# Plonky3/Plonky3-recursion

Hardware: AMD Instinct MI355X
Metric: prove_next_layer ms + Poseidon2 perms/s, KoalaBear 2^20-row circuit, 1/8 GPU (lower is better)
Workload: dtype u32 Montgomery (31-bit prime field, degree-4 extension); Poseidon2 hashing as exact integers in f64; 1 GPU; prove_next_layer (verifier-circuit run on the device + prove_all_tables) of the synthetic koala-bear 2^20-row recursion layer: tables const/public/alu/poseidon2/recompose, FRI blowup 4, arity<=4, 54 queries, 15-bit PoW; circuit inputs + NextLayerPrepCache resident in HBM; field=koala-bear, log_height=20, independent_proofs=1, proof_bytes=612900, parallelism=1 independent proofs, one per GPU, no data-path collective

## Files before the change

### __graft_entry__.py

```python
import os
import subprocess
import sys
import time

ROOT = os.path.dirname(os.path.abspath(__file__))
CSRC = os.path.join(ROOT, "plonky3_recursion_amd", "csrc")
LIB = os.path.join(ROOT, "plonky3_recursion_amd", "libp3r_hip.so")
KNOBS_LIB = os.path.join(ROOT, "plonky3_recursion_amd", "knobs", "libp3r_hip.so")
HIP_SOURCES = ["p3r_core.hip", "tu_lde.hip", "tu_open.hip", "tu_fri.hip", "tu_quotient.hip", "tu_logup.hip", "tu_mmcs4.hip", "prep_device.hip"]


def _stale(target, deps):
    if not os.path.exists(target):
        return True
    t = os.path.getmtime(target)
    return any(os.path.getmtime(d) > t for d in deps)


def _deps_of(obj):
    dep = obj + ".d"
    if not os.path.exists(dep):
        return None
    txt = open(dep).read().replace("\\\n", " ")
    return [p for p in txt.split(":", 1)[1].split() if p]


def build():
    hipcc = os.environ.get("HIPCC", "/opt/rocm/bin/hipcc")
    flags = ["-O3", "-std=c++17", "--offload-arch=gfx950", "-fPIC", "-pthread"]
    objdir = os.path.join(CSRC, ".build")
    os.makedirs(objdir, exist_ok=True)
    os.makedirs(os.path.dirname(KNOBS_LIB), exist_ok=True)
    shared = ["prep_device.hip", "tu_open.hip", "tu_fri.hip", "tu_quotient.hip", "tu_logup.hip", "tu_mmcs4.hip"]
    knobbed = ["p3r_core.hip", "tu_lde.hip"]
    units = [(src, src + ".o", []) for src in HIP_SOURCES]
    units += [(src, src.replace(".hip", ".knobs.o"), ["-DP3R_TUNING_KNOBS"]) for src in knobbed]
    test_only = ["tu_prims_test.hip", "tu_p2f_test.hip", "tu_field_test.hip"]
    units += [(src, src.replace(".hip", ".knobs.o"), ["-DP3R_TUNING_KNOBS"]) for src in test_only]
    pending = []
    for src, objname, extra in units:
        obj = os.path.join(objdir, objname)
        deps = _deps_of(obj)
        if deps is None or not all(os.path.exists(d) for d in deps) or _stale(obj, deps):
            pending.append((obj, [hipcc] + flags + extra + ["-MD", "-MF", obj + ".d", "-c", "-o", obj, os.path.join(CSRC, src)]))
    pending.sort(key=lambda job: 0 if "p3r_core" in os.path.basename(job[0]) else 1)
    running, failed = [], None
    max_jobs = max(1, min(len(pending), (os.cpu_count() or 2)))
    while pending or running:
        while pending and len(running) < max_jobs:
            obj, cmd = pending.pop(0)
            running.append((obj, subprocess.Popen(cmd, cwd=CSRC)))
        done = [job for job in running if job[1].poll() is not None]
# ... 104 lines not shown
```

### plonky3_recursion_amd/csrc/circuit_impl.hip.h

```cpp

#include "circuit_host.h"

namespace {

template <class PP, int D = 4>
__device__ __forceinline__ typename CircuitExt<PP, D>::type w_load(const uint32_t* __restrict__ w, uint32_t id) {
  typename CircuitExt<PP, D>::type e;
  if constexpr (D == 4) {
    const uint4 v = *reinterpret_cast<const uint4*>(w + (size_t)id * 4);
    e.c[0] = Fp<PP>::raw(v.x); e.c[1] = Fp<PP>::raw(v.y); e.c[2] = Fp<PP>::raw(v.z); e.c[3] = Fp<PP>::raw(v.w);
  } else {
#pragma unroll
    for (int k = 0; k < D; ++k) e.c[k] = Fp<PP>::raw(w[(size_t)id * D + k]);
  }
  return e;
}
template <class PP, int D = 4>
__device__ __forceinline__ void w_store(uint32_t* __restrict__ w, uint32_t id, const typename CircuitExt<PP, D>::type& e) {
  if constexpr (D == 4) {
    *reinterpret_cast<uint4*>(w + (size_t)id * 4) = make_uint4(e.c[0].v, e.c[1].v, e.c[2].v, e.c[3].v);
  } else {
#pragma unroll
    for (int k = 0; k < D; ++k) w[(size_t)id * D + k] = e.c[k].v;
  }
// ... 24 lines not shown
struct RunArgs {
  const RunOp* light;
  const RunP2* p2;
  const RunP2B* p2b;
  uint32_t* w;
  const uint32_t* ext;
  uint32_t* alu_values;
  uint32_t* rec_values;
  uint32_t* p2_inputs;
  size_t p2_h;
  uint8_t* p2_flags;
  uint32_t* p2_seed;
  uint32_t* p2_out;
  const int32_t* pd_slot;
  const uint32_t* siblings;
  const uint32_t* rc;
  const uint32_t* diag;
  uint32_t* err;
  const uint32_t* light_off;
  const RunSchedule::P2Seg* p2segs;
  const uint32_t* p2seg_off;
  const RunP2W* p2w;
  uint32_t* p2w_inputs;
  size_t p2w_h;
  uint8_t* p2w_flags;
  uint32_t* p2w_out;
  const int32_t* pdw_slot;
  const uint32_t* siblings_w;
  const uint32_t* rcw;
  const RunSchedule::P2Seg* p2wsegs;
  const uint32_t* p2wseg_off;
};
// ... 92 lines not shown
      }
      w_put<PP, D>(w, op.out, v, chk_out, err, op.op_idx);
      break;
    }
    default: break;
  }
}

template <class PP>
__device__ __forceinline__ void run_p2_segment(const RunArgs& A, RunSchedule::P2Seg seg, int j, bool live) {
  using F = Fp<PP>;
  using E = Fp4<PP>;
  uint32_t* __restrict__ w = A.w;
  uint32_t* err = A.err;
  if (!live) seg.n = 0;
  const CoopRc<PP> rcs = coop_load_rc<PP>(A.rc, j);
  const F diag_j = F::raw(A.diag[j]);
  F carried = F::zero();
  RunP2 next = seg.n ? A.p2[seg.first] : RunP2{};
  for (uint32_t k = 0; k < seg.n; ++k) {
    const RunP2 q = next;
    if (k + 1 < seg.n) next = A.p2[seg.first + k + 1];
    const bool new_start = q.flags & 1, merkle = q.flags & 2;
    F s = F::zero();
    if (!new_start && (!merkle || j < 8)) s = k ? carried : F::raw(A.p2_out[(size_t)q.prev_row * 16 + j]);
    const int32_t slot = A.pd_slot[q.row];
    if (merkle && slot >= 0 && j >= 8) s = F::raw(A.siblings[(size_t)slot * 8 + (j - 8)]);
    const uint32_t in_w = q.in[j >> 2];
    if (in_w != kNoW) s = F::raw(w[(size_t)in_w * 4 + (j & 3)]);
    bool bit = false;
    if (q.bit_w != kNoW) {
      const E v = w_load<PP>(w, q.bit_w);
// ... 5 lines not shown
      if (merkle && bit) s = F::raw(other);
    }
    A.p2_inputs[(size_t)j * A.p2_h + q.row] = s.v;
    if (j == 0) {
      A.p2_flags[q.row] = q.flags & 1;
      A.p2_flags[A.p2_h + q.row] = (q.flags >> 1) & 1;
      A.p2_flags[2 * A.p2_h + q.row] = bit;
      uint32_t seed = 0;
      if (q.idx_w != kNoW) {
        const E v = w_load<PP>(w, q.idx_w);
        if (v.c[1].v | v.c[2].v | v.c[3].v) run_error(err, q.op_idx, RUN_ERR_INDEX_SUM);
        seed = v.c[0].v;
      }
      A.p2_seed[q.row] = seed;
    }
    s = coop_permute<PP>(s, j, diag_j, rcs);
    carried = s;
    A.p2_out[(size_t)q.row * 16 + j] = s.v;
    const uint32_t n_out = (q.flags >> 8) & 7;
    const uint32_t l = (uint32_t)j >> 2;
    if (l < n_out && q.out[l] != kNoW) {
      uint32_t* slot_w = w + (size_t)q.out[l] * 4 + (j & 3);
      if (q.flags & (1u << (4 + l))) { if (*slot_w != s.v) run_error(err, q.op_idx, RUN_ERR_CONFLICT); }
      else *slot_w = s.v;
    }
  }
}

template <class PP>
__device__ __forceinline__ void run_p2w_segment(const RunArgs& A, RunSchedule::P2Seg seg, int j, bool live) {
  using F = Fp<PP>;
// ... 46 lines not shown
    const uint32_t l = (uint32_t)j >> 2;
    if (l < n_out && q.out[l] != kNoW) {
      uint32_t* slot_w = w + (size_t)q.out[l] * 4 + (j & 3);
      if (q.flags & (1u << (16 + l))) { if (*slot_w != s.v) run_error(err, q.op_idx, RUN_ERR_CONFLICT); }
      else *slot_w = s.v;
    }
  }
}

template <class PP, int D>
__device__ __forceinline__ void run_p2_segment_base(const RunArgs& A, RunSchedule::P2Seg seg, int j, bool live) {
  using F = Fp<PP>;
  uint32_t* __restrict__ w = A.w;
  uint32_t* err = A.err;
  if (!live) seg.n = 0;
  const CoopRc<PP> rcs = coop_load_rc<PP>(A.rc, j);
  const F diag_j = F::raw(A.diag[j]);
  F carried = F::zero();
  for (uint32_t k = 0; k < seg.n; ++k) {
    const RunP2B& q = A.p2b[seg.first + k];
    const uint32_t flags = q.flags;
    const bool new_start = flags & 1, merkle = flags & 2;
    F s = F::zero();
    if (!new_start && (!merkle || j < 8)) s = k ? carried : F::raw(A.p2_out[(size_t)q.prev_row * 16 + j]);
    const int32_t slot = A.pd_slot[q.row];
    if (merkle && slot >= 0 && j >= 8) s = F::raw(A.siblings[(size_t)slot * 8 + (j - 8)]);
    const uint32_t in_w = q.in[j];
    if (in_w != kNoW) s = F::raw(w[(size_t)in_w * D]);
    if (!merkle && j == 8 && q.absorb_len) s = s + F::from_canonical(q.absorb_len);
    bool bit = false;
    if (q.bit_w != kNoW) {
      const auto v = w_load<PP, D>(w, q.bit_w);
// ... 8 lines not shown
    A.p2_inputs[(size_t)j * A.p2_h + q.row] = s.v;
    if (j == 0) {
      A.p2_flags[q.row] = flags & 1;
      A.p2_flags[A.p2_h + q.row] = (flags >> 1) & 1;
      A.p2_flags[2 * A.p2_h + q.row] = bit;
      uint32_t seed = 0;
      if (q.idx_w != kNoW) {
        const auto v = w_load<PP, D>(w, q.idx_w);
        uint32_t high = 0;
        for (int c = 1; c < D; ++c) high |= v.c[c].v;
        if (high) run_error(err, q.op_idx, RUN_ERR_INDEX_SUM);
        seed = v.c[0].v;
      }
      A.p2_seed[q.row] = seed;
    }
    s = coop_permute<PP>(s, j, diag_j, rcs);
    carried = s;
    A.p2_out[(size_t)q.row * 16 + j] = s.v;
    const uint32_t n_out = (flags >> 8) & 31;
    if ((uint32_t)j < n_out && q.out[j] != kNoW) {
      uint32_t* slot_w = w + (size_t)q.out[j] * D;
      if (q.check_mask & (1u << j)) {
        bool same = slot_w[0] == s.v;
        for (int c = 1; c < D; ++c) same = same && slot_w[c] == 0;
        if (!same) run_error(err, q.op_idx, RUN_ERR_CONFLICT);
      } else {
        slot_w[0] = s.v;
        for (int c = 1; c < D; ++c) slot_w[c] = 0;
      }
    }
  }
// ... 512 lines not shown
    P3R_HIP(fill_async(ctx->stream, p2w_flags + p2w_h, 0, 3 * p2w_h));
    d->seed.alloc(p2w_h);
    P3R_HIP(fill_async(ctx->stream, d->seed.p, 0, p2w_h * 4));
    p2w_inputs = d->inputs->d;
    T->p2w = std::move(d);
  }
  {
    ProfScope ps(ctx, "run_levels");
    RunArgs A{};
    A.light = reinterpret_cast<const RunOp*>(C->d_light.p);
    A.p2 = reinterpret_cast<const RunP2*>(C->d_p2.p);
    A.p2b = reinterpret_cast<const RunP2B*>(C->d_p2.p);
    A.w = w.p; A.ext = C->d_ext.p; A.alu_values = T->alu_values.p; A.rec_values = T->recompose_values.p;
    A.p2_inputs = p2_inputs; A.p2_h = p2_h; A.p2_flags = p2_flags; A.p2_seed = p2_seed; A.p2_out = p2_out.p;
    A.pd_slot = reinterpret_cast<const int32_t*>(d_slot.p); A.siblings = d_sib.p;
    A.rc = ctx->rc.p; A.diag = ctx->p2_diag.p; A.err = err.p;
    A.light_off = C->d_light_off.p; A.p2seg_off = C->d_p2seg_off.p;
    A.p2segs = reinterpret_cast<const RunSchedule::P2Seg*>(C->d_p2segs.p);
    const bool has_w32 = !S.p2wseg_off.empty();
    if (has_w32) {
      A.p2w = reinterpret_cast<const RunP2W*>(C->d_p2w.p);
      A.p2w_inputs = p2w_inputs; A.p2w_h = p2w_h; A.p2w_flags = p2w_flags; A.p2w_out = p2w_out.p;
      A.pdw_slot = reinterpret_cast<const int32_t*>(in->slot_w.p); A.siblings_w = in->sib_w.p;
      A.rcw = ctx->rc.p + p2_num_constants<PP>();
      A.p2wsegs = reinterpret_cast<const RunSchedule::P2Seg*>(C->d_p2wsegs.p);
      A.p2wseg_off = C->d_p2wseg_off.p;
    }
    dispatch_ext_degree<PP>((int)ext_d, [&](auto dc) {
    constexpr int DD = decltype(dc)::value;
    for (const auto& seg : S.segments) {
      if (seg.narrow) {
// ... 110 lines not shown
```

### plonky3_recursion_amd/csrc/context.h

```cpp
#pragma once
#include <hip/hip_runtime.h>

#include <algorithm>
#include <array>
#include <atomic>
#include <cstdarg>
#include <cstdio>
#include <cstring>
#include <exception>
#include <functional>
#include <map>
#include <memory>
#include <chrono>
#include <mutex>
#include <stdexcept>
#include <string>
#include <thread>
#include <tuple>
#include <vector>

#include "../../include/p3r.h"
#include "error.h"
#include "field.h"
#include "poseidon2.h"
// ... 422 lines not shown
  p3r_config cfg{};
  std::shared_ptr<p3r::DevPool> pool = std::make_shared<p3r::DevPool>();
  bool prof_enabled = false;
  std::vector<p3r::ProfRec> prof;
  std::vector<std::pair<std::string, double>> stage_ms;
  std::string cur_stage;
  double cur_stage_t0 = 0;
  int partial_rounds = 0;
  hipStream_t stream = nullptr;
  int n_cus = 256;
  p3r::DevBuf rc;
  p3r::DevBuf rc_f64;
  const double* rcd() const { return reinterpret_cast<const double*>(rc_f64.p); }
  size_t rcd_w32_at = 0;
  const double* rcd_w32() const { return rcd() + rcd_w32_at; }
  p3r::DevBuf p2_diag;
  std::vector<uint32_t> rc_canonical;
  std::vector<uint8_t> fri_log_arities;
  p3r::ProofLayout proof_layout;
  std::vector<uint32_t> rc_mont_host;
  std::string err;
  bool w32_diag_builtin = false;
  bool w32_unacknowledged = false;
  uint64_t zk_nonce = 0;
  uint32_t zk_key[8] = {0, 0, 0, 0, 0, 0, 0, 0};
  std::vector<uint8_t> pending_proof;
  p3r::HostStage stage;
  p3r::HostLanding landing;
  p3r::HostPost post;
  std::map<std::string, p3r::DevBuf> const_tables;

// ... 19 lines not shown
```

### plonky3_recursion_amd/csrc/kernels_coop.hip.h

```cpp
#pragma once
#include "kernels.hip.h"

namespace p3r {

template <int CTRL>
__device__ __forceinline__ uint32_t dpp(uint32_t v) {
  return (uint32_t)__builtin_amdgcn_update_dpp(0, (int)v, CTRL, 0xF, 0xF, false);
}
constexpr int DPP_QUAD_NEXT1 = 0x39;
constexpr int DPP_QUAD_NEXT2 = 0x4E;
constexpr int DPP_QUAD_NEXT3 = 0x93;
constexpr int DPP_ROW_ROR1 = 0x121, DPP_ROW_ROR2 = 0x122, DPP_ROW_ROR4 = 0x124, DPP_ROW_ROR8 = 0x128;

template <class F>
__device__ __forceinline__ F coop_external(F x) {
  F b = F::raw(dpp<DPP_QUAD_NEXT1>(x.v)), c = F::raw(dpp<DPP_QUAD_NEXT2>(x.v)), d = F::raw(dpp<DPP_QUAD_NEXT3>(x.v));
  F ab = x + b;
  F y = ab.dbl() + b + (c + d);
  F t = y + F::raw(dpp<DPP_ROW_ROR4>(y.v));
  t = t + F::raw(dpp<DPP_ROW_ROR8>(t.v));
  return y + t;
}
template <class F>
__device__ __forceinline__ F coop_row_sum(F x) {
  F t = x + F::raw(dpp<DPP_ROW_ROR8>(x.v));
  t = t + F::raw(dpp<DPP_ROW_ROR4>(t.v));
  t = t + F::raw(dpp<DPP_ROW_ROR2>(t.v));
  return t + F::raw(dpp<DPP_ROW_ROR1>(t.v));
}

constexpr int DPP_QUAD_BCAST0 = 0x00;
__device__ __forceinline__ uint32_t coop_bcast0(uint32_t x0) {
  uint32_t q = dpp<DPP_QUAD_BCAST0>(x0);
  q |= dpp<DPP_ROW_ROR4>(q);
  return q | dpp<DPP_ROW_ROR8>(q);
}

template <class PP>
struct CoopRc {
  uint32_t full[2 * P2_HALF_FULL];
  uint32_t part[PP::PARTIAL_ROUNDS];
};
template <class PP>
__device__ __forceinline__ CoopRc<PP> coop_load_rc(const uint32_t* __restrict__ rc, int elem) {
  CoopRc<PP> c;
#pragma unroll
  for (int r = 0; r < P2_HALF_FULL; ++r) c.full[r] = rc[r * P2_WIDTH + elem];
#pragma unroll
  for (int r = 0; r < PP::PARTIAL_ROUNDS; ++r) c.part[r] = rc[P2_HALF_FULL * P2_WIDTH + r];
#pragma unroll
  for (int r = 0; r < P2_HALF_FULL; ++r)
    c.full[P2_HALF_FULL + r] = rc[P2_HALF_FULL * P2_WIDTH + PP::PARTIAL_ROUNDS + r * P2_WIDTH + elem];
  return c;
}

template <class PP>
__device__ __forceinline__ Fp<PP> coop_permute(Fp<PP> s, int elem, Fp<PP> diag, const CoopRc<PP>& rc) {
  using F = Fp<PP>;
  s = coop_external(s);
#pragma unroll
  for (int r = 0; r < P2_HALF_FULL; ++r) {
    s = p2_sbox<PP>(s + F::raw(rc.full[r]));
    s = coop_external(s);
  }
#pragma unroll
  for (int r = 0; r < PP::PARTIAL_ROUNDS; ++r) {
    const F rest = coop_row_sum(elem == 0 ? F::zero() : s);
    const F sb = p2_sbox<PP>(s + F::raw(rc.part[r]));
    const F sum = rest + F::raw(coop_bcast0(elem == 0 ? sb.v : 0u));
    s = (elem == 0 ? sb : s) * diag + sum;
  }
#pragma unroll
  for (int r = 0; r < P2_HALF_FULL; ++r) {
    s = p2_sbox<PP>(s + F::raw(rc.full[P2_HALF_FULL + r]));
    s = coop_external(s);
  }
  return s;
}

template <class PP>
__global__ void __launch_bounds__(kBlock)
k_mmcs_hash_rows_strided_coop(const uint32_t* const* __restrict__ cols, int wtot, size_t h, size_t stride,
                              uint32_t* __restrict__ dig, const uint32_t* __restrict__ rc,
                              const uint32_t* __restrict__ diag) {
  using F = Fp<PP>;
  const size_t gid = (size_t)blockIdx.x * kBlock + threadIdx.x;
  const size_t row = gid >> 4;
  const int e = (int)(gid & 15);
  const bool live = row < h;
  const F d = F::raw(diag[e]);
  const CoopRc<PP> rcs = coop_load_rc<PP>(rc, e);
  F s = F::zero();
  for (int g = 0; g < wtot; g += P2_RATE) {
    if (live && e < P2_RATE && g + e < wtot) s = F::raw(cols[g + e][row * stride]);
    s = coop_permute<PP>(s, e, d, rcs);
  }
  if (live && e < P2_DIGEST) dig[(size_t)e * h + row] = s.v;
}

constexpr int kSubtreeBlock = 1024;
constexpr int kSubtreeNodes = 256;
constexpr int kSubtreeLevels = 8;
struct SubtreeArgs {
  const uint32_t* in;
  uint32_t n_in;
  uint32_t local;
  int n_levels;
  uint32_t* out[kSubtreeLevels];
  const uint32_t* inj[kSubtreeLevels];
  uint32_t* t_state;
  uint32_t* t_beta;
  uint32_t* t_cap;
  int t_dc;
};

template <class PP>
__device__ __forceinline__ void fri_transcript_step(int j, uint32_t root_word, uint32_t* __restrict__ state,
                                                    uint32_t* __restrict__ beta_out, uint32_t* __restrict__ cap_out,
                                                    const CoopRc<PP>& rc, const uint32_t* __restrict__ diag, int dc = 4) {
  using F = Fp<PP>;
  F s = j < P2_RATE ? F::raw(root_word) : F::raw(state[j]);
  if (j < P2_RATE) cap_out[j] = s.v;
  if (j == P2_RATE) s += F::from_canonical(P2_RATE);
  s = coop_permute<PP>(s, j, F::raw(diag[j]), rc);
  state[j] = s.v;
  if (j >= P2_RATE - dc && j < P2_RATE) beta_out[7 - j] = s.v;
}
template <class PP>
__global__ void __launch_bounds__(kSubtreeBlock)
k_mmcs_subtree(SubtreeArgs a, const uint32_t* __restrict__ rc, const uint32_t* __restrict__ diag) {
  using F = Fp<PP>;
  __shared__ uint32_t buf[2][P2_DIGEST * kSubtreeNodes / 2];
  const int elem = threadIdx.x & 15;
  const uint32_t group = threadIdx.x >> 4, k = elem & 7;
  const F d = F::raw(diag[elem]);
  const CoopRc<PP> rcs = coop_load_rc<PP>(rc, elem);
  uint32_t n = a.n_in < a.local ? a.n_in : a.local;
  uint32_t n_glob = a.n_in, first = blockIdx.x * n;
#pragma unroll
  for (int l = 0; l < kSubtreeLevels; ++l) {
    if (l < a.n_levels) {
      const uint32_t nn = n / 2, nn_glob = n_glob / 2, first_out = first / 2;
      const uint32_t* cur = buf[(l + 1) & 1];
      uint32_t* nxt = buf[l & 1];
      for (uint32_t node = group; node < nn; node += blockDim.x / 16) {
        const uint32_t child = 2 * node + (elem >> 3);
        F s = F::raw(l == 0 ? a.in[(size_t)k * n_glob + first + child] : cur[k * n + child]);
        s = coop_permute<PP>(s, elem, d, rcs);
        if (a.inj[l]) {
          if (elem >= P2_DIGEST) s = F::raw(a.inj[l][(size_t)k * nn_glob + first_out + node]);
          s = coop_permute<PP>(s, elem, d, rcs);
        }
        if (elem < P2_DIGEST) {
          nxt[k * nn + node] = s.v;
          a.out[l][(size_t)k * nn_glob + first_out + node] = s.v;
        }
      }
      __syncthreads();
      n = nn;
      n_glob = nn_glob;
      first = first_out;
    }
  }
  if (a.t_state && threadIdx.x < P2_WIDTH) {
    const uint32_t* root = buf[(a.n_levels - 1) & 1];
    fri_transcript_step<PP>((int)threadIdx.x, threadIdx.x < P2_RATE ? root[threadIdx.x] : 0u, a.t_state, a.t_beta,
                            a.t_cap, rcs, diag, a.t_dc ? a.t_dc : 4);
  }
}

template <class PP>
__global__ void __launch_bounds__(64)
k_fri_transcript_step(const uint32_t* __restrict__ root , uint32_t* __restrict__ state ,
                      uint32_t* __restrict__ beta_out , uint32_t* __restrict__ cap_out ,
                      const uint32_t* __restrict__ rc, const uint32_t* __restrict__ diag, int dc) {
  const int j = threadIdx.x;
  if (j >= P2_WIDTH) return;
  fri_transcript_step<PP>(j, j < P2_RATE ? root[j] : 0u, state, beta_out, cap_out, coop_load_rc<PP>(rc, j), diag, dc);
}



template <class F>
__device__ __forceinline__ F coop32_pair_sum(F t) {
  const auto r = __builtin_amdgcn_permlane16_swap(t.v, t.v, false, false);
  return F::raw(r[0]) + F::raw(r[1]);
}
template <class F>
__device__ __forceinline__ F coop32_external(F x) {
  const F b = F::raw(dpp<DPP_QUAD_NEXT1>(x.v)), c = F::raw(dpp<DPP_QUAD_NEXT2>(x.v)), d = F::raw(dpp<DPP_QUAD_NEXT3>(x.v));
  const F ab = x + b;
  const F y = ab.dbl() + b + (c + d);
  F t = y + F::raw(dpp<DPP_ROW_ROR4>(y.v));
// ... 57 lines not shown
```

### plonky3_recursion_amd/csrc/mmcs_impl.hip.h

```cpp

namespace {

template <class PP>
void hash_rows(p3r_ctx* ctx, const std::vector<std::vector<const p3r_dmat*>>& classes,
               const std::vector<uint32_t*>& digs) {
  std::vector<HashRowsJob> jobs;
  for (size_t c = 0; c < classes.size(); ++c) {
    std::vector<const uint32_t*> cols;
    for (const p3r_dmat* m : classes[c])
      for (size_t k = 0; k < m->w; ++k) cols.push_back(m->d + k * m->h);
    HashRowsJob j{};
    j.cols = col_table(ctx, cols);
    j.dig = digs[c];
    j.h = classes[c][0]->h;
    j.wtot = (int)cols.size();
    jobs.push_back(j);
  }
  std::stable_sort(jobs.begin(), jobs.end(),
                   [](const HashRowsJob& a, const HashRowsJob& b) { return a.wtot > b.wtot; });
  uint32_t blocks = 0;
  double perms = 0;
  for (auto& j : jobs) {
    j.block0 = blocks;
    blocks += blocks_for(j.h);
// ... 66 lines not shown
    push_layer(tree, lv.padded_next);
    a.out[a.n_levels] = tree->layers.back().p;
    a.inj[a.n_levels] = injected_at(inject, lv);
    ++a.n_levels;
  }
  if (step && tree->layer_n.back() == 1 && n == local) {
    a.t_state = step->state;
    a.t_beta = step->beta;
    a.t_cap = step->cap;
    a.t_dc = step->dc;
    step->done = true;
  }
  ProfScope ps(ctx, "mmcs_compress");
  const unsigned lanes = (unsigned)std::min<size_t>(std::max<size_t>(local * 8, 64), kSubtreeBlock);
  hipLaunchKernelGGL(k_mmcs_subtree<PP>, dim3((unsigned)(n / local)), dim3(lanes), 0, ctx->stream, a,
                     ctx->rc.p, ctx->p2_diag.p);
  P3R_HIP(hipGetLastError());
  return (size_t)a.n_levels;
}

inline void mmcs_begin(p3r_ctx* ctx, p3r_tree* tree, const std::vector<size_t>& heights) {
  const size_t hmax = *std::max_element(heights.begin(), heights.end());
  tree->arity = ctx->cfg.mmcs_arity == 4 ? 4 : 2;
  tree->log_max_h = log2_exact(hmax, "matrix height");
  tree->cap_height = (int)ctx->cfg.cap_height;
  tree->levels = tree->arity == 4 ? mmcs4_schedule(heights) : mmcs2_schedule(heights, tree->log_max_h, tree->cap_height);
  tree->layers.clear();
  tree->layer_n.clear();
  const size_t n0 = tree->arity == 4 ? mmcs4_padded_len(hmax) : hmax;
  push_layer(tree, n0);
  if (n0 != hmax) P3R_HIP(fill_async(ctx->stream, tree->layers[0].p, 0, P2_DIGEST * n0 * 4));
// ... 19 lines not shown
    tree->layers.push_back(std::move(next));
    tree->layer_n.push_back(lv.padded_next);
  }
}

template <class PP>
void mmcs_hash_rows_strided(p3r_ctx* ctx, p3r_tree* tree, const std::vector<const uint32_t*>& cols, size_t rows, size_t stride) {
  const uint32_t* const* dcols = col_table(ctx, cols);
  uint32_t* dig = tree->layers[0].p;
  if (tree->arity == 4) {
    mmcs4_hash_rows_strided<PP>(ctx, dcols, (int)cols.size(), rows, stride, dig, tree->layer_n[0]);
  } else {
    ProfScope ps(ctx, "mmcs_hash_rows_strided");
    if (rows <= coop_max_leaf_rows())
      hipLaunchKernelGGL(k_mmcs_hash_rows_strided_coop<PP>, dim3(blocks_for(rows * 16)), dim3(kBlock), 0,
                         ctx->stream, dcols, (int)cols.size(), rows, stride, dig, ctx->rc.p, ctx->p2_diag.p);
    else
      hipLaunchKernelGGL(k_mmcs_hash_rows_strided<PP>, dim3(blocks_for(rows)), dim3(kBlock), 0, ctx->stream,
                         dcols, (int)cols.size(), rows, stride, dig, ctx->rcd());
  }
  P3R_HIP(hipGetLastError());
}

inline std::vector<uint32_t> mmcs_cap_mont(p3r_ctx* ctx, const p3r_tree* tree) {
  const size_t cap_n = tree->layer_n.back();
  std::vector<uint32_t> soa(P2_DIGEST * cap_n), cap(P2_DIGEST * cap_n);
  P3R_HIP(fetch_small(ctx, tree->layers.back().p, soa.size(), soa.data()));
  for (size_t j = 0; j < cap_n; ++j)
    for (int k = 0; k < P2_DIGEST; ++k) cap[j * P2_DIGEST + k] = soa[(size_t)k * cap_n + j];
  return cap;
}
// ... 150 lines not shown
```

### plonky3_recursion_amd/csrc/p3r_core.hip

```cpp
#include "context.h"
#include "kernels.hip.h"
#include "kernels_stark.hip.h"
#include "kernels_coop.hip.h"
#include "tu_api.h"
#include "profile.h"
#include "run_schedule.h"
#include "prep_device.h"
#include "host_abi.h"

#include <sys/random.h>

#include <algorithm>
#include <cerrno>
#include <future>
#include <numeric>
#include <unordered_map>

using namespace p3r;

namespace {

thread_local std::string g_create_error;

template <class Fn>
// ... 163 lines not shown
  ctx->rcd_w32_at = nrc;
  {
    const size_t nrcw = p2w_num_rc<PP>();
    const uint32_t* w = src + nrc;
    rcd.insert(rcd.end(), w, w + nrcw);
    for (int i = 0; i < P2W_WIDTH; ++i) {
      const uint32_t d = w[nrcw + i];
      rcd.push_back(d > PP::P / 2 ? (double)d - (double)PP::P : (double)d);
    }
    const uint32_t* builtin = PP::FIELD_ID == 0 ? kDefaultDiagW32_koala_bear : kDefaultDiagW32_baby_bear;
    const bool is_builtin = std::equal(builtin, builtin + P2W_WIDTH, w + nrcw) && !tuning_knob("P3R_W32_GENERAL_DIAG");
    ctx->w32_diag_builtin = is_builtin;
  }
  ctx->rc_f64.alloc(2 * rcd.size());
  P3R_HIP(copy_sync(ctx->stream, ctx->rc_f64.p, rcd.data(), rcd.size() * 8, hipMemcpyHostToDevice));
  {
    auto inv2k = [](int k) { return F::from_u64(uint64_t(1) << k).inv(); };
    const F two = F::from_canonical(2), three = F::from_canonical(3), four = F::from_canonical(4);
    F d[16] = {-two, F::one(), two, inv2k(1), three, four, -inv2k(1), -three, -four, inv2k(8), inv2k(3), inv2k(24),
               -inv2k(8), -inv2k(3), -inv2k(4), -inv2k(24)};
    if (PP::FIELD_ID == 1) {
      F b[16] = {-two, F::one(), two, inv2k(1), three, four, -inv2k(1), -three, -four, inv2k(8), inv2k(2), inv2k(3),
                 inv2k(27), -inv2k(8), -inv2k(4), -inv2k(27)};
      for (int i = 0; i < 16; ++i) d[i] = b[i];
    }
    uint32_t dm[16];
    for (int i = 0; i < 16; ++i) dm[i] = d[i].v;
    ctx->p2_diag.alloc(16);
    P3R_HIP(copy_sync(ctx->stream, ctx->p2_diag.p, dm, sizeof dm, hipMemcpyHostToDevice));
  }
  ctx->partial_rounds = PP::PARTIAL_ROUNDS;
  ctx->cfg.poseidon2_rc = nullptr;
  ctx->w32_unacknowledged = (!ctx->cfg.poseidon2_w32_rc || !ctx->cfg.poseidon2_w32_diag) && !(ctx->cfg.ext_choices & P3R_EXT_UNPINNED_W32_DEFAULTS);
  if (ctx->w32_unacknowledged && ctx->cfg.mmcs_arity == 4)
    fail(P3R_EINVAL, "mmcs_arity = 4 with poseidon2_w32_rc / poseidon2_w32_diag NULL: the built-in width-32 constants are self-generated, "
                     "not upstream's - pass the caller's, or acknowledge with P3R_EXT_UNPINNED_W32_DEFAULTS");
  ctx->cfg.poseidon2_w32_rc = nullptr;
  ctx->cfg.poseidon2_w32_diag = nullptr;
  if (ctx->cfg.fri_log_arities) ctx->fri_log_arities.assign(ctx->cfg.fri_log_arities, ctx->cfg.fri_log_arities + ctx->cfg.fri_log_arities_len);
  ctx->cfg.fri_log_arities = nullptr;
  if (!ctx->proof_layout.set(ctx->cfg.proof_layout, ctx->cfg.proof_layout_len))
    fail(P3R_EINVAL, "proof_layout must be 18 bytes: three permutations batch[5] | fri[5] | opened[8]");
  ctx->cfg.proof_layout = nullptr;
  lde_init<PP>(ctx);
}
// ... 936 lines not shown
```

### plonky3_recursion_amd/csrc/prove_impl.hip.h

```cpp
#include "host_transcript.h"
#include "kernels_stark.hip.h"
#include "kernels_fri_reduce.hip.h"
#include "kernels_zk.hip.h"
#include "open_impl.hip.h"

struct p3r_prep {
  std::vector<p3r::AirParams> airs;
  std::vector<std::unique_ptr<p3r_dmat>> traces;
  std::vector<std::unique_ptr<p3r_dmat>> evals;
  std::vector<std::unique_ptr<p3r_dmat>> ldes;
  std::vector<size_t> heights;
  int zk_codewords = -1;
  const p3r_dmat* committed(size_t i) const { return evals.empty() ? traces[i].get() : evals[i].get(); }
  std::unique_ptr<p3r_tree> tree;
  std::vector<uint32_t> cap_canonical;
};

namespace {

template <class PP, int DC = 4>
EW<DC> to_e4(const typename Chal<PP, DC>::type& e) { return e4_store<PP, DC>(e); }

template <class PP, int DC = 4>
std::vector<typename Chal<PP, DC>::type> download_ef(p3r_ctx* ctx, const uint32_t* dev, size_t count) {
// ... 770 lines not shown
      int log_next = next_h < heights.size() ? heights[next_h] : -1;
      int la = fri_log_arity(ctx->fri_log_arities, phases.size(), (int)cfg.max_log_arity, log_cur, log_final, log_next);
      if (la < 0) fail(P3R_EINVAL, "fri_log_arities does not fit the proof: phase %zu at height 2^%d", phases.size(), log_cur);
      if (la > 4) fail(P3R_EUNSUPPORTED, "max_log_arity > 4 is not supported");
      const size_t arity = size_t(1) << la, rows = (size_t(1) << log_cur) >> la;
      Phase ph{la, rows};
      commit_phase_leaves(ph, log_cur);
      const size_t pi = phases.size();
      if (pi >= kMaxPhases) fail(P3R_EUNSUPPORTED, "more than %zu FRI commit phases", kMaxPhases);
      TranscriptStep step{d_tstate.p, d_betas + DC * pi, d_caps + P2_DIGEST * pi};
      step.dc = DC;
      mmcs_build_levels<PP>(ctx, ph.tree.get(), nullptr, device_transcript ? &step : nullptr);
      if (device_transcript) {
        if (!step.done)
          hipLaunchKernelGGL(k_fri_transcript_step<PP>, dim3(1), dim3(64), 0, ctx->stream, ph.tree->layers.back().p,
                             step.state, step.beta, step.cap, ctx->rc.p, ctx->p2_diag.p, DC);
      } else {
        ph.cap = mmcs_cap_mont(ctx, ph.tree.get());
        for (uint32_t v : ph.cap) ch.observe(F::raw(v));
        commit_pow_witnesses.push_back(grind_witness<PP>(ctx, ch, (int)cfg.commit_pow_bits));
        const E beta = ch.sample_ext();
        uint32_t bw[DC];
        for (int k = 0; k < DC; ++k) bw[k] = beta.c[k].v;
        P3R_HIP(ctx->stage.upload(ctx->stream, d_betas + DC * pi, bw, sizeof bw));
      }
      DevBuf out(DC * rows);
      FriFoldArgs fa{};
      fa.in = folded.p; fa.out = out.p; fa.rows = rows; fa.log_rows = log_cur - la;
      fa.beta = d_betas + DC * pi;
      const bool roll = next_h < heights.size() && heights[next_h] == log_cur - la;
      fa.roll = roll ? ros[heights[next_h]].second.p : nullptr;
// ... 306 lines not shown
```

Before: 25.99 ms.

## Port cooperative 16-lane Poseidon2 permutation from Montgomery u32 to exact FP64 arithmetic

Replaces the integer Montgomery cooperative Poseidon2 permutation, used by the circuit runner, MMCS leaf hashing, subtree compression and the FRI transcript, with an FP64 version. Values stay in doubles across DPP lane shuffles, and a compile-time walk checks that every intermediate stays below 2^53. The partial rounds are restructured so the diagonal multiply uses a fract-based reduction and the lane-0 s-box is pipelined. This aims to move Poseidon2 onto the FP64 units and cut the cost of Montgomery multiplies. In exchange, each shuffle now needs two DPP ops instead of one, register pressure rises, and shared buffers double in size.

```diff
diff --git a/__graft_entry__.py b/__graft_entry__.py
--- a/__graft_entry__.py
+++ b/__graft_entry__.py
@@ -35,7 +35,7 @@
     knobbed = ["p3r_core.hip", "tu_lde.hip"]
     units = [(src, src + ".o", []) for src in HIP_SOURCES]
     units += [(src, src.replace(".hip", ".knobs.o"), ["-DP3R_TUNING_KNOBS"]) for src in knobbed]
-    test_only = ["tu_prims_test.hip", "tu_p2f_test.hip", "tu_field_test.hip"]
+    test_only = ["tu_prims_test.hip", "tu_p2f_test.hip", "tu_coop_test.hip", "tu_field_test.hip"]
     units += [(src, src.replace(".hip", ".knobs.o"), ["-DP3R_TUNING_KNOBS"]) for src in test_only]
     pending = []
     for src, objname, extra in units:
diff --git a/plonky3_recursion_amd/csrc/circuit_impl.hip.h b/plonky3_recursion_amd/csrc/circuit_impl.hip.h
--- a/plonky3_recursion_amd/csrc/circuit_impl.hip.h
+++ b/plonky3_recursion_amd/csrc/circuit_impl.hip.h
@@ -62,8 +62,7 @@
   uint32_t* p2_out;
   const int32_t* pd_slot;
   const uint32_t* siblings;
-  const uint32_t* rc;
-  const uint32_t* diag;
+  const double* rcd;
   uint32_t* err;
   const uint32_t* light_off;
   const RunSchedule::P2Seg* p2segs;
@@ -186,8 +185,8 @@
   uint32_t* __restrict__ w = A.w;
   uint32_t* err = A.err;
   if (!live) seg.n = 0;
-  const CoopRc<PP> rcs = coop_load_rc<PP>(A.rc, j);
-  const F diag_j = F::raw(A.diag[j]);
+  const CoopFRc<PP, double> rcs = coopf_load_rc<PP>(A.rcd, j);
+  const P2FSboxK<PP> SK = p2f_sbox_consts<PP>();
   F carried = F::zero();
   RunP2 next = seg.n ? A.p2[seg.first] : RunP2{};
   for (uint32_t k = 0; k < seg.n; ++k) {
@@ -223,7 +222,7 @@
       }
       A.p2_seed[q.row] = seed;
     }
-    s = coop_permute<PP>(s, j, diag_j, rcs);
+    s = coop_permute_words<PP>(s, j, rcs, SK);
     carried = s;
     A.p2_out[(size_t)q.row * 16 + j] = s.v;
     const uint32_t n_out = (q.flags >> 8) & 7;
@@ -300,8 +299,8 @@
   uint32_t* __restrict__ w = A.w;
   uint32_t* err = A.err;
   if (!live) seg.n = 0;
-  const CoopRc<PP> rcs = coop_load_rc<PP>(A.rc, j);
-  const F diag_j = F::raw(A.diag[j]);
+  const CoopFRc<PP, double> rcs = coopf_load_rc<PP>(A.rcd, j);
+  const P2FSboxK<PP> SK = p2f_sbox_consts<PP>();
   F carried = F::zero();
   for (uint32_t k = 0; k < seg.n; ++k) {
     const RunP2B& q = A.p2b[seg.first + k];
@@ -340,7 +339,7 @@
       }
       A.p2_seed[q.row] = seed;
     }
-    s = coop_permute<PP>(s, j, diag_j, rcs);
+    s = coop_permute_words<PP>(s, j, rcs, SK);
     carried = s;
     A.p2_out[(size_t)q.row * 16 + j] = s.v;
     const uint32_t n_out = (flags >> 8) & 31;
@@ -883,7 +882,7 @@
     A.w = w.p; A.ext = C->d_ext.p; A.alu_values = T->alu_values.p; A.rec_values = T->recompose_values.p;
     A.p2_inputs = p2_inputs; A.p2_h = p2_h; A.p2_flags = p2_flags; A.p2_seed = p2_seed; A.p2_out = p2_out.p;
     A.pd_slot = reinterpret_cast<const int32_t*>(d_slot.p); A.siblings = d_sib.p;
-    A.rc = ctx->rc.p; A.diag = ctx->p2_diag.p; A.err = err.p;
+    A.rcd = ctx->rcd(); A.err = err.p;
     A.light_off = C->d_light_off.p; A.p2seg_off = C->d_p2seg_off.p;
     A.p2segs = reinterpret_cast<const RunSchedule::P2Seg*>(C->d_p2segs.p);
     const bool has_w32 = !S.p2wseg_off.empty();
diff --git a/plonky3_recursion_amd/csrc/context.h b/plonky3_recursion_amd/csrc/context.h
--- a/plonky3_recursion_amd/csrc/context.h
+++ b/plonky3_recursion_amd/csrc/context.h
@@ -460,7 +460,6 @@
   const double* rcd() const { return reinterpret_cast<const double*>(rc_f64.p); }
   size_t rcd_w32_at = 0;
   const double* rcd_w32() const { return rcd() + rcd_w32_at; }
-  p3r::DevBuf p2_diag;
   std::vector<uint32_t> rc_canonical;
   std::vector<uint8_t> fri_log_arities;
   p3r::ProofLayout proof_layout;
diff --git a/plonky3_recursion_amd/csrc/kernels_coop.hip.h b/plonky3_recursion_amd/csrc/kernels_coop.hip.h
--- a/plonky3_recursion_amd/csrc/kernels_coop.hip.h
+++ b/plonky3_recursion_amd/csrc/kernels_coop.hip.h
@@ -1,5 +1,6 @@
 #pragma once
 #include "kernels.hip.h"
+#include "poseidon2_coop_f64.hip.h"
 
 namespace p3r {
 
@@ -7,20 +8,7 @@
 __device__ __forceinline__ uint32_t dpp(uint32_t v) {
   return (uint32_t)__builtin_amdgcn_update_dpp(0, (int)v, CTRL, 0xF, 0xF, false);
 }
-constexpr int DPP_QUAD_NEXT1 = 0x39;
-constexpr int DPP_QUAD_NEXT2 = 0x4E;
-constexpr int DPP_QUAD_NEXT3 = 0x93;
-constexpr int DPP_ROW_ROR1 = 0x121, DPP_ROW_ROR2 = 0x122, DPP_ROW_ROR4 = 0x124, DPP_ROW_ROR8 = 0x128;
 
-template <class F>
-__device__ __forceinline__ F coop_external(F x) {
-  F b = F::raw(dpp<DPP_QUAD_NEXT1>(x.v)), c = F::raw(dpp<DPP_QUAD_NEXT2>(x.v)), d = F::raw(dpp<DPP_QUAD_NEXT3>(x.v));
-  F ab = x + b;
-  F y = ab.dbl() + b + (c + d);
-  F t = y + F::raw(dpp<DPP_ROW_ROR4>(y.v));
-  t = t + F::raw(dpp<DPP_ROW_ROR8>(t.v));
-  return y + t;
-}
 template <class F>
 __device__ __forceinline__ F coop_row_sum(F x) {
   F t = x + F::raw(dpp<DPP_ROW_ROR8>(x.v));
@@ -29,7 +17,6 @@
   return t + F::raw(dpp<DPP_ROW_ROR1>(t.v));
 }
 
-constexpr int DPP_QUAD_BCAST0 = 0x00;
 __device__ __forceinline__ uint32_t coop_bcast0(uint32_t x0) {
   uint32_t q = dpp<DPP_QUAD_BCAST0>(x0);
   q |= dpp<DPP_ROW_ROR4>(q);
@@ -37,65 +24,26 @@
 }
 
 template <class PP>
-struct CoopRc {
-  uint32_t full[2 * P2_HALF_FULL];
-  uint32_t part[PP::PARTIAL_ROUNDS];
-};
-template <class PP>
-__device__ __forceinline__ CoopRc<PP> coop_load_rc(const uint32_t* __restrict__ rc, int elem) {
-  CoopRc<PP> c;
-#pragma unroll
-  for (int r = 0; r < P2_HALF_FULL; ++r) c.full[r] = rc[r * P2_WIDTH + elem];
-#pragma unroll
-  for (int r = 0; r < PP::PARTIAL_ROUNDS; ++r) c.part[r] = rc[P2_HALF_FULL * P2_WIDTH + r];
-#pragma unroll
-  for (int r = 0; r < P2_HALF_FULL; ++r)
-    c.full[P2_HALF_FULL + r] = rc[P2_HALF_FULL * P2_WIDTH + PP::PARTIAL_ROUNDS + r * P2_WIDTH + elem];
-  return c;
-}
-
-template <class PP>
-__device__ __forceinline__ Fp<PP> coop_permute(Fp<PP> s, int elem, Fp<PP> diag, const CoopRc<PP>& rc) {
-  using F = Fp<PP>;
-  s = coop_external(s);
-#pragma unroll
-  for (int r = 0; r < P2_HALF_FULL; ++r) {
-    s = p2_sbox<PP>(s + F::raw(rc.full[r]));
-    s = coop_external(s);
-  }
-#pragma unroll
-  for (int r = 0; r < PP::PARTIAL_ROUNDS; ++r) {
-    const F rest = coop_row_sum(elem == 0 ? F::zero() : s);
-    const F sb = p2_sbox<PP>(s + F::raw(rc.part[r]));
-    const F sum = rest + F::raw(coop_bcast0(elem == 0 ? sb.v : 0u));
-    s = (elem == 0 ? sb : s) * diag + sum;
-  }
-#pragma unroll
-  for (int r = 0; r < P2_HALF_FULL; ++r) {
-    s = p2_sbox<PP>(s + F::raw(rc.full[P2_HALF_FULL + r]));
-    s = coop_external(s);
-  }
-  return s;
+__device__ __forceinline__ Fp<PP> coop_permute_words(Fp<PP> s, int elem, const CoopFRc<PP, double>& rc, const P2FSboxK<PP>& K) {
+  return Fp<PP>::raw(p2f_store<PP>(coop_permute_f64<PP, false>(p2f_load<PP>(s.v), elem, rc, K)));
 }
 
 template <class PP>
 __global__ void __launch_bounds__(kBlock)
 k_mmcs_hash_rows_strided_coop(const uint32_t* const* __restrict__ cols, int wtot, size_t h, size_t stride,
-                              uint32_t* __restrict__ dig, const uint32_t* __restrict__ rc,
-                              const uint32_t* __restrict__ diag) {
-  using F = Fp<PP>;
+                              uint32_t* __restrict__ dig, const double* __restrict__ rcd) {
   const size_t gid = (size_t)blockIdx.x * kBlock + threadIdx.x;
   const size_t row = gid >> 4;
   const int e = (int)(gid & 15);
   const bool live = row < h;
-  const F d = F::raw(diag[e]);
-  const CoopRc<PP> rcs = coop_load_rc<PP>(rc, e);
-  F s = F::zero();
+  const CoopFRc<PP, double> rcs = coopf_load_rc<PP>(rcd, e);
+  const P2FSboxK<PP> K = p2f_sbox_consts<PP>();
+  double s = 0.0;
   for (int g = 0; g < wtot; g += P2_RATE) {
-    if (live && e < P2_RATE && g + e < wtot) s = F::raw(cols[g + e][row * stride]);
-    s = coop_permute<PP>(s, e, d, rcs);
+    if (live && e < P2_RATE && g + e < wtot) s = p2f_load<PP>(cols[g + e][row * stride]);
+    s = coop_permute_f64<PP>(s, e, rcs, K);
   }
-  if (live && e < P2_DIGEST) dig[(size_t)e * h + row] = s.v;
+  if (live && e < P2_DIGEST) dig[(size_t)e * h + row] = p2f_store<PP>(s);
 }
 
 constexpr int kSubtreeBlock = 1024;
@@ -115,45 +63,44 @@
 };
 
 template <class PP>
-__device__ __forceinline__ void fri_transcript_step(int j, uint32_t root_word, uint32_t* __restrict__ state,
+__device__ __forceinline__ void fri_transcript_step(int j, double root_word, uint32_t* __restrict__ state,
                                                     uint32_t* __restrict__ beta_out, uint32_t* __restrict__ cap_out,
-                                                    const CoopRc<PP>& rc, const uint32_t* __restrict__ diag, int dc = 4) {
-  using F = Fp<PP>;
-  F s = j < P2_RATE ? F::raw(root_word) : F::raw(state[j]);
-  if (j < P2_RATE) cap_out[j] = s.v;
-  if (j == P2_RATE) s += F::from_canonical(P2_RATE);
-  s = coop_permute<PP>(s, j, F::raw(diag[j]), rc);
-  state[j] = s.v;
-  if (j >= P2_RATE - dc && j < P2_RATE) beta_out[7 - j] = s.v;
+                                                    const CoopFRc<PP, double>& rc, const P2FSboxK<PP>& K, int dc = 4) {
+  double s = j < P2_RATE ? root_word : p2f_load<PP>(state[j]);
+  if (j < P2_RATE) cap_out[j] = p2f_store<PP>(s);
+  if (j == P2_RATE) s += (double)P2_RATE;
+  const uint32_t v = p2f_store<PP>(coop_permute_f64<PP>(s, j, rc, K));
+  state[j] = v;
+  if (j >= P2_RATE - dc && j < P2_RATE) beta_out[7 - j] = v;
 }
 template <class PP>
 __global__ void __launch_bounds__(kSubtreeBlock)
-k_mmcs_subtree(SubtreeArgs a, const uint32_t* __restrict__ rc, const uint32_t* __restrict__ diag) {
-  using F = Fp<PP>;
-  __shared__ uint32_t buf[2][P2_DIGEST * kSubtreeNodes / 2];
+k_mmcs_subtree(SubtreeArgs a, const double* __restrict__ rcd) {
+  __shared__ double buf[2][P2_DIGEST * kSubtreeNodes / 2];
   const int elem = threadIdx.x & 15;
   const uint32_t group = threadIdx.x >> 4, k = elem & 7;
-  const F d = F::raw(diag[elem]);
-  const CoopRc<PP> rcs = coop_load_rc<PP>(rc, elem);
+  const CoopFRc<PP, double> rcs = coopf_load_rc<PP>(rcd, elem);
+  const P2FSboxK<PP> K = p2f_sbox_consts<PP>();
   uint32_t n = a.n_in < a.local ? a.n_in : a.local;
   uint32_t n_glob = a.n_in, first = blockIdx.x * n;
 #pragma unroll
   for (int l = 0; l < kSubtreeLevels; ++l) {
     if (l < a.n_levels) {
       const uint32_t nn = n / 2, nn_glob = n_glob / 2, first_out = first / 2;
-      const uint32_t* cur = buf[(l + 1) & 1];
-      uint32_t* nxt = buf[l & 1];
+      const double* cur = buf[(l + 1) & 1];
+      double* nxt = buf[l & 1];
       for (uint32_t node = group; node < nn; node += blockDim.x / 16) {
         const uint32_t child = 2 * node + (elem >> 3);
-        F s = F::raw(l == 0 ? a.in[(size_t)k * n_glob + first + child] : cur[k * n + child]);
-        s = coop_permute<PP>(s, elem, d, rcs);
+        double s;
+        if (l == 0) s = coop_permute_f64<PP, false>(p2f_load<PP>(a.in[(size_t)k * n_glob + first + child]), elem, rcs, K);
+        else s = coop_permute_f64<PP, true>(cur[k * n + child], elem, rcs, K);
         if (a.inj[l]) {
-          if (elem >= P2_DIGEST) s = F::raw(a.inj[l][(size_t)k * nn_glob + first_out + node]);
-          s = coop_permute<PP>(s, elem, d, rcs);
+          if (elem >= P2_DIGEST) s = p2f_load<PP>(a.inj[l][(size_t)k * nn_glob + first_out + node]);
+          s = coop_permute_f64<PP, true>(s, elem, rcs, K);
         }
         if (elem < P2_DIGEST) {
-          nxt[k * nn + node] = s.v;
-          a.out[l][(size_t)k * nn_glob + first_out + node] = s.v;
+          nxt[k * nn + node] = s;
+          a.out[l][(size_t)k * nn_glob + first_out + node] = p2f_store<PP>(s);
         }
       }
       __syncthreads();
@@ -163,9 +110,9 @@
     }
   }
   if (a.t_state && threadIdx.x < P2_WIDTH) {
-    const uint32_t* root = buf[(a.n_levels - 1) & 1];
-    fri_transcript_step<PP>((int)threadIdx.x, threadIdx.x < P2_RATE ? root[threadIdx.x] : 0u, a.t_state, a.t_beta,
-                            a.t_cap, rcs, diag, a.t_dc ? a.t_dc : 4);
+    const double* root = buf[(a.n_levels - 1) & 1];
+    fri_transcript_step<PP>((int)threadIdx.x, threadIdx.x < P2_RATE ? root[threadIdx.x] : 0.0, a.t_state, a.t_beta,
+                            a.t_cap, rcs, K, a.t_dc ? a.t_dc : 4);
   }
 }
 
@@ -173,10 +120,11 @@
 __global__ void __launch_bounds__(64)
 k_fri_transcript_step(const uint32_t* __restrict__ root , uint32_t* __restrict__ state ,
                       uint32_t* __restrict__ beta_out , uint32_t* __restrict__ cap_out ,
-                      const uint32_t* __restrict__ rc, const uint32_t* __restrict__ diag, int dc) {
+                      const double* __restrict__ rcd, int dc) {
   const int j = threadIdx.x;
   if (j >= P2_WIDTH) return;
-  fri_transcript_step<PP>(j, j < P2_RATE ? root[j] : 0u, state, beta_out, cap_out, coop_load_rc<PP>(rc, j), diag, dc);
+  fri_transcript_step<PP>(j, j < P2_RATE ? p2f_load<PP>(root[j]) : 0.0, state, beta_out, cap_out, coopf_load_rc<PP>(rcd, j),
+                          p2f_sbox_consts<PP>(), dc);
 }
 
 
diff --git a/plonky3_recursion_amd/csrc/mmcs_impl.hip.h b/plonky3_recursion_amd/csrc/mmcs_impl.hip.h
--- a/plonky3_recursion_amd/csrc/mmcs_impl.hip.h
+++ b/plonky3_recursion_amd/csrc/mmcs_impl.hip.h
@@ -104,7 +104,7 @@
   ProfScope ps(ctx, "mmcs_compress");
   const unsigned lanes = (unsigned)std::min<size_t>(std::max<size_t>(local * 8, 64), kSubtreeBlock);
   hipLaunchKernelGGL(k_mmcs_subtree<PP>, dim3((unsigned)(n / local)), dim3(lanes), 0, ctx->stream, a,
-                     ctx->rc.p, ctx->p2_diag.p);
+                     ctx->rcd());
   P3R_HIP(hipGetLastError());
   return (size_t)a.n_levels;
 }
@@ -154,7 +154,7 @@
     ProfScope ps(ctx, "mmcs_hash_rows_strided");
     if (rows <= coop_max_leaf_rows())
       hipLaunchKernelGGL(k_mmcs_hash_rows_strided_coop<PP>, dim3(blocks_for(rows * 16)), dim3(kBlock), 0,
-                         ctx->stream, dcols, (int)cols.size(), rows, stride, dig, ctx->rc.p, ctx->p2_diag.p);
+                         ctx->stream, dcols, (int)cols.size(), rows, stride, dig, ctx->rcd());
     else
       hipLaunchKernelGGL(k_mmcs_hash_rows_strided<PP>, dim3(blocks_for(rows)), dim3(kBlock), 0, ctx->stream,
                          dcols, (int)cols.size(), rows, stride, dig, ctx->rcd());
diff --git a/plonky3_recursion_amd/csrc/p3r_core.hip b/plonky3_recursion_amd/csrc/p3r_core.hip
--- a/plonky3_recursion_amd/csrc/p3r_core.hip
+++ b/plonky3_recursion_amd/csrc/p3r_core.hip
@@ -201,21 +201,6 @@
   }
   ctx->rc_f64.alloc(2 * rcd.size());
   P3R_HIP(copy_sync(ctx->stream, ctx->rc_f64.p, rcd.data(), rcd.size() * 8, hipMemcpyHostToDevice));
-  {
-    auto inv2k = [](int k) { return F::from_u64(uint64_t(1) << k).inv(); };
-    const F two = F::from_canonical(2), three = F::from_canonical(3), four = F::from_canonical(4);
-    F d[16] = {-two, F::one(), two, inv2k(1), three, four, -inv2k(1), -three, -four, inv2k(8), inv2k(3), inv2k(24),
-               -inv2k(8), -inv2k(3), -inv2k(4), -inv2k(24)};
-    if (PP::FIELD_ID == 1) {
-      F b[16] = {-two, F::one(), two, inv2k(1), three, four, -inv2k(1), -three, -four, inv2k(8), inv2k(2), inv2k(3),
-                 inv2k(27), -inv2k(8), -inv2k(4), -inv2k(27)};
-      for (int i = 0; i < 16; ++i) d[i] = b[i];
-    }
-    uint32_t dm[16];
-    for (int i = 0; i < 16; ++i) dm[i] = d[i].v;
-    ctx->p2_diag.alloc(16);
-    P3R_HIP(copy_sync(ctx->stream, ctx->p2_diag.p, dm, sizeof dm, hipMemcpyHostToDevice));
-  }
   ctx->partial_rounds = PP::PARTIAL_ROUNDS;
   ctx->cfg.poseidon2_rc = nullptr;
   ctx->w32_unacknowledged = (!ctx->cfg.poseidon2_w32_rc || !ctx->cfg.poseidon2_w32_diag) && !(ctx->cfg.ext_choices & P3R_EXT_UNPINNED_W32_DEFAULTS);
diff --git a/plonky3_recursion_amd/csrc/poseidon2_coop_f64.hip.h b/plonky3_recursion_amd/csrc/poseidon2_coop_f64.hip.h
--- /dev/null
+++ b/plonky3_recursion_amd/csrc/poseidon2_coop_f64.hip.h
@@ -0,0 +1,174 @@
+#pragma once
+#include "poseidon2_f64.hip.h"
+
+namespace p3r {
+
+constexpr int DPP_QUAD_NEXT1 = 0x39;
+constexpr int DPP_QUAD_NEXT2 = 0x4E;
+constexpr int DPP_QUAD_NEXT3 = 0x93;
+constexpr int DPP_QUAD_BCAST0 = 0x00;
+constexpr int DPP_ROW_ROR1 = 0x121, DPP_ROW_ROR2 = 0x122, DPP_ROW_ROR4 = 0x124, DPP_ROW_ROR8 = 0x128;
+
+#pragma clang fp contract(off)
+
+template <class PP>
+constexpr double coopf_factor(int i) {
+  return i == 0 ? 0.0 : p2f_lane_factor<PP>(i);
+}
+
+template <class PP, class V>
+struct CoopFRc {
+  V full[2 * P2_HALF_FULL];
+  double part[PP::PARTIAL_ROUNDS];
+  V m, k15;
+};
+
+template <class PP>
+constexpr int coopf_walk() {
+  using u64 = unsigned long long;
+  constexpr u64 EXACT = u64(1) << 53, SBOX_IN = u64(1) << 38, P = PP::P;
+  constexpr u64 SBOX_OUT = (7 * P + 9) / 10, RED = P / 2 + 2, FULL_OUT = 35 * SBOX_OUT;
+  if (35 * P + (P - 1) >= SBOX_IN) return 1;
+  if (FULL_OUT + (P - 1) >= SBOX_IN) return 2;
+  u64 S = FULL_OUT, X = FULL_OUT + (P - 1), REST = RED;
+  if (15 * FULL_OUT >= EXACT) return 3;
+  for (int r = 0; r < PP::PARTIAL_ROUNDS; ++r) {
+    const int at = 1000 * (r + 1);
+    if (X >= SBOX_IN) return at + 1;
+    u64 W = 0;
+    for (int i = 1; i < P2_WIDTH; ++i) {
+      const P2FLane L = p2f_lane<PP>(i);
+      u64 prod = 0;
+      if (L.form == P2F_DYADIC) {
+        if (L.k > 8 || L.k > PP::TWO_ADICITY || S >= (EXACT >> L.k)) return at + 10 * i + 2;
+        prod = ((S + (u64(1) << L.k) - 1) >> L.k) + P;
+      } else {
+        prod = u64(L.d < 0 ? -L.d : L.d) * S;
+      }
+      if (prod + REST >= EXACT) return at + 10 * i + 3;
+      const u64 w = 15 * S + prod;
+      if (w >= EXACT) return at + 10 * i + 4;
+      W += w;
+    }
+    if (W >= EXACT) return at + 5;
+    X = REST + (P - 1) + SBOX_OUT;
+    REST = 15 * SBOX_OUT + RED;
+    S = RED + SBOX_OUT;
+    if (REST >= EXACT) return at + 6;
+  }
+  if ((X > S ? X : S) + (P - 1) >= SBOX_IN) return 100000;
+  if (FULL_OUT >= (u64(1) << 36)) return 100001;
+  return 0;
+}
+static_assert(coopf_walk<KoalaBearParams>() == 0, "KoalaBear: the cooperative FP64 permutation leaves exact arithmetic");
+static_assert(coopf_walk<BabyBearParams>() == 0, "BabyBear: the cooperative FP64 permutation leaves exact arithmetic");
+
+template <class O>
+P3R_HD typename O::V coopf_external(const O& o, typename O::V x) {
+  using V = typename O::V;
+  const V b = o.template dpp<DPP_QUAD_NEXT1>(x), c = o.template dpp<DPP_QUAD_NEXT2>(x), d = o.template dpp<DPP_QUAD_NEXT3>(x);
+  const V ab = x + b, bcd = b + (c + d);
+  const V y = o.fma(ab, o.splat(2.0), bcd);
+  V t = y + o.template dpp<DPP_ROW_ROR4>(y);
+  t = t + o.template dpp<DPP_ROW_ROR8>(t);
+  return y + t;
+}
+template <class O>
+P3R_HD typename O::V coopf_row_sum(const O& o, typename O::V x) {
+  using V = typename O::V;
+  V t = x + o.template dpp<DPP_ROW_ROR8>(x);
+  t = t + o.template dpp<DPP_ROW_ROR4>(t);
+  t = t + o.template dpp<DPP_ROW_ROR2>(t);
+  return t + o.template dpp<DPP_ROW_ROR1>(t);
+}
+
+template <class PP, bool CARRIED, class O>
+P3R_HD typename O::V coopf_permute(const O& o, typename O::V s, const CoopFRc<PP, typename O::V>& rc, const P2FSboxK<PP>& K) {
+  using V = typename O::V;
+  constexpr int R = PP::PARTIAL_ROUNDS;
+  if (CARRIED) s = o.template reduce<PP>(s);
+  s = coopf_external(o, s);
+#pragma unroll
+  for (int r = 0; r < P2_HALF_FULL; ++r) {
+    s = o.template sbox<PP>(s + rc.full[r], K);
+    s = coopf_external(o, s);
+  }
+  V x = o.bcast0(s) + o.splat(rc.part[0]);
+  V rest = o.template reduce<PP>(coopf_row_sum(o, o.lane0(o.splat(0.0), s)));
+  V u = s, sb = o.splat(0.0);
+#pragma unroll
+  for (int r = 0; r < R; ++r) {
+    const V sv = r == 0 ? u : u + sb;
+    const V t = sv * rc.m;
+    const V p = o.fma(o.neg(o.fract(t)), o.splat(P2F64<PP>::P), t);
+    const V A = o.template reduce<PP>(coopf_row_sum(o, o.fma(sv, rc.k15, p)));
+    u = o.template reduce<PP>(p + rest);
+    sb = o.template sbox<PP>(x, K);
+    x = (rest + o.splat(r + 1 < R ? rc.part[r + 1 < R ? r + 1 : r] : 0.0)) - sb;
+    rest = o.fma(sb, o.splat(15.0), A);
+  }
+  s = o.lane0(x, u + sb);
+#pragma unroll
+  for (int r = 0; r < P2_HALF_FULL; ++r) {
+    s = o.template sbox<PP>(s + rc.full[P2_HALF_FULL + r], K);
+    s = coopf_external(o, s);
+  }
+  return s;
+}
+
+#if defined(__HIPCC__)
+struct CoopFLane {
+  using V = double;
+  bool is0;
+  template <int CTRL>
+  __device__ __forceinline__ double dpp(double v) const {
+    const uint64_t b = __builtin_bit_cast(uint64_t, v);
+    const uint32_t lo = (uint32_t)__builtin_amdgcn_update_dpp(0, (int)(uint32_t)b, CTRL, 0xF, 0xF, true);
+    const uint32_t hi = (uint32_t)__builtin_amdgcn_update_dpp(0, (int)(uint32_t)(b >> 32), CTRL, 0xF, 0xF, true);
+    return __builtin_bit_cast(double, (uint64_t)hi << 32 | lo);
+  }
+  __device__ __forceinline__ double splat(double c) const { return c; }
+  __device__ __forceinline__ double fma(double a, double b, double c) const { return __builtin_fma(a, b, c); }
+  __device__ __forceinline__ double neg(double a) const { return -a; }
+  __device__ __forceinline__ double fract(double a) const { return p2f_fract(a); }
+  __device__ __forceinline__ double lane0(double at0, double other) const { return is0 ? at0 : other; }
+  __device__ __forceinline__ double bcast0(double v) const {
+    uint64_t q = __builtin_bit_cast(uint64_t, dpp<DPP_QUAD_BCAST0>(is0 ? v : 0.0));
+    q |= __builtin_bit_cast(uint64_t, dpp<DPP_ROW_ROR4>(__builtin_bit_cast(double, q)));
+    q |= __builtin_bit_cast(uint64_t, dpp<DPP_ROW_ROR8>(__builtin_bit_cast(double, q)));
+    return __builtin_bit_cast(double, q);
+  }
+  template <class PP>
+  __device__ __forceinline__ double reduce(double a) const { return p2f_reduce<PP>(a); }
+  template <class PP>
+  __device__ __forceinline__ double sbox(double a, const P2FSboxK<PP>& K) const { return p2f_sbox<PP>(a, K); }
+};
+
+template <class PP>
+__device__ __forceinline__ CoopFRc<PP, double> coopf_load_rc(const double* __restrict__ rcd, int elem) {
+  CoopFRc<PP, double> c;
+#pragma unroll
+  for (int r = 0; r < P2_HALF_FULL; ++r) c.full[r] = rcd[r * P2_WIDTH + elem];
+#pragma unroll
+  for (int r = 0; r < PP::PARTIAL_ROUNDS; ++r) c.part[r] = rcd[P2_HALF_FULL * P2_WIDTH + r];
+#pragma unroll
+  for (int r = 0; r < P2_HALF_FULL; ++r)
+    c.full[P2_HALF_FULL + r] = rcd[P2_HALF_FULL * P2_WIDTH + PP::PARTIAL_ROUNDS + r * P2_WIDTH + elem];
+  double m = 0.0;
+#pragma unroll
+  for (int i = 1; i < P2_WIDTH; ++i)
+    if (elem == i) m = coopf_factor<PP>(i);
+  c.m = m;
+  c.k15 = elem == 0 ? 0.0 : 15.0;
+  return c;
+}
+
+template <class PP, bool CARRIED = true>
+__device__ __forceinline__ double coop_permute_f64(double s, int elem, const CoopFRc<PP, double>& rc, const P2FSboxK<PP>& K) {
+  return coopf_permute<PP, CARRIED>(CoopFLane{elem == 0}, s, rc, K);
+}
+#endif
+
+#pragma clang fp contract(fast)
+
+}
diff --git a/plonky3_recursion_amd/csrc/prove_impl.hip.h b/plonky3_recursion_amd/csrc/prove_impl.hip.h
--- a/plonky3_recursion_amd/csrc/prove_impl.hip.h
+++ b/plonky3_recursion_amd/csrc/prove_impl.hip.h
@@ -808,7 +808,7 @@
       if (device_transcript) {
         if (!step.done)
           hipLaunchKernelGGL(k_fri_transcript_step<PP>, dim3(1), dim3(64), 0, ctx->stream, ph.tree->layers.back().p,
-                             step.state, step.beta, step.cap, ctx->rc.p, ctx->p2_diag.p, DC);
+                             step.state, step.beta, step.cap, ctx->rcd(), DC);
       } else {
         ph.cap = mmcs_cap_mont(ctx, ph.tree.get());
         for (uint32_t v : ph.cap) ch.observe(F::raw(v));
```

New measurement: 26.21 ms. About the same (+0.8%).
